# fredli74/hashbox

Hardware: AMD Instinct MI355X
Metric: device-resident GiB/s chunked+hashed at 1/2/4/8 MI355X; % HBM roofline (higher is better)
Workload: dtype u8

## Files before the change

hashbox_amd/csrc/hbx_kernels.hip:

```cpp
#include <type_traits>
#include <utility>

#include "hbx_device.h"

using namespace hbx;

namespace {

constexpr int kK1Threads = 1024;

struct RunAgg {
  uint32_t ah, jh, af, jf;
};
__device__ __forceinline__ RunAgg run_aggregates(const uint32_t (&v)[16]) {
  RunAgg r;
  uint32_t a = 0, j = 0;
#pragma unroll
  for (int k = 0; k < 8; k++) {
    a = dot4(v[k], 0x01010101u, a);
    j = dot4(v[k], jw(k), j);
  }
  r.ah = a;
  r.jh = j;
#pragma unroll
// ... 670 lines not shown
    }
    md5_compress(h, m);
  }
}

__device__ void md5_block_at(const uint8_t* c, uint32_t len, uint32_t (&h)[4], uint32_t b) {
  const uint32_t sh = (uint32_t)reinterpret_cast<uintptr_t>(c) & 3u;
  g_u32* va = gptr32(c - sh);
  const uint32_t base = b ? 16u * b - 2u : 0u;
  uint32_t v[17];
#pragma unroll
  for (int j = 0; j < 17; j++) v[j] = va[base + (uint32_t)j];
  uint32_t m[16];
#pragma unroll
  for (int j = 0; j < 16; j++) {
    const uint32_t dw = alignbyte(v[j + 1], v[j], sh);
    const uint32_t d0 = j >= 2 ? alignbyte(v[j - 1], v[j - 2], sh) : 0u;
    m[j] = b ? dw : (j == 0 ? 0u : j == 1 ? bswap32(len) : d0);
  }
  md5_compress(h, m);
}

template <int G>
struct Coop {
  static constexpr uint32_t C = 64u / G;
  static constexpr uint32_t Row = 16u * G + 16u;
  static constexpr uint32_t Half = 64u * Row;
  static constexpr uint32_t WaveLds = 2u * Half;
  static constexpr uint32_t BPS = G / 4u;
};
constexpr uint32_t kCoopWaveLds = Coop<16>::WaveLds;

__device__ __forceinline__ uint64_t shfl64(uint64_t v, uint32_t src_lane) {
  const int lo = __builtin_amdgcn_ds_bpermute((int)(src_lane << 2), (int)(uint32_t)v);
  const int hi = __builtin_amdgcn_ds_bpermute((int)(src_lane << 2), (int)(uint32_t)(v >> 32));
  return ((uint64_t)(uint32_t)hi << 32) | (uint32_t)lo;
}

template <int G>
__device__ __forceinline__ void coop_write(uint8_t* wl, uint32_t wr, uint32_t half, const u32x4 (&Gs)[G]) {
#pragma unroll
  for (int q = 0; q < G; q++)
    *reinterpret_cast<u32x4*>(wl + wr + half * Coop<G>::Half + Coop<G>::C * Coop<G>::Row * (uint32_t)q) = Gs[q];
}

template <int G>
__device__ __forceinline__ void coop_load(u32x4 (&Gs)[G], const uint64_t (&Q)[G], uint32_t st, uint32_t t,
                                          uint32_t ngr) {
  const uint32_t g = min((uint32_t)G * st + t, ngr - 1u);
  const uint64_t off = 16ull * (g - t);
#pragma unroll
  for (int q = 0; q < G; q++) Gs[q] = md5_load(gptr128(Q[q] + off));
}

template <int G>
__device__ __forceinline__ void coop_hash(const uint8_t* wl, uint32_t rd, uint32_t half, uint32_t s, uint32_t R,
                                          uint32_t (&h)[4]) {
  const uint8_t* hb = wl + rd + half * Coop<G>::Half;
#pragma unroll
  for (int u = 0; u < (int)Coop<G>::BPS; u++) {
    const uint32_t blk = Coop<G>::BPS * s + (uint32_t)u;
    if (blk >= R) break;
    u32x4 W[4];
#pragma unroll
    for (int i = 0; i < 4; i++) W[i] = *reinterpret_cast<const u32x4*>(hb + 16u * (4u * u + (uint32_t)i));
    const uint32_t m[16] = {W[0].x, W[0].y, W[0].z, W[0].w, W[1].x, W[1].y, W[1].z, W[1].w,
                            W[2].x, W[2].y, W[2].z, W[2].w, W[3].x, W[3].y, W[3].z, W[3].w};
    md5_compress(h, m);
  }
}

template <int G>
__device__ void md5_coop(uint8_t* wl, const uint8_t* c, uint32_t (&h)[4], uint32_t b1, uint32_t R) {
  static_assert(G == 16, "stage of 4 blocks");
  const uint32_t lane = threadIdx.x & 63u;
  const uint64_t S = reinterpret_cast<uint64_t>(c) + 64ull * b1 - 8ull;
  const uint32_t ngr = 4u * R;
  const uint32_t t = lane % (uint32_t)G, sub = lane / (uint32_t)G;
  uint64_t Q[G];
#pragma unroll
  for (int q = 0; q < G; q++) Q[q] = shfl64(S, Coop<G>::C * (uint32_t)q + sub) + 16ull * t;
  const uint32_t wr = sub * Coop<G>::Row + 16u * t;
  const uint32_t rd = lane * Coop<G>::Row;
  const uint32_t nst = (ngr + (uint32_t)G - 1u) / (uint32_t)G;
  constexpr uint32_t BPS = Coop<G>::BPS;
  u32x4 GA[G], GB[G];
  coop_load<G>(GA, Q, 0u, t, ngr);
  coop_load<G>(GB, Q, 1u, t, ngr);
  coop_write<G>(wl, wr, 0u, GA);
  coop_load<G>(GA, Q, 2u, t, ngr);
  auto stage = [&](auto half_c, uint32_t s, u32x4(&Gn)[G]) {
    constexpr uint32_t HALF = decltype(half_c)::value;
    coop_write<G>(wl, wr, HALF ^ 1u, Gn);
    coop_load<G>(Gn, Q, min(s + 3u, nst - 1u), t, ngr);
    coop_hash<G>(wl, rd, HALF, s, R, h);
  };
  for (uint32_t s = 0; BPS * s < R; s += 2u) {
    stage(std::integral_constant<uint32_t, 0>{}, s, GB);
    stage(std::integral_constant<uint32_t, 1>{}, s + 1u, GA);
  }
}

}

struct alignas(16) Chain {
  uint64_t src;
  uint32_t len;
  uint32_t next;
  uint32_t h[4];
  uint64_t out;
  uint64_t pad;
};
constexpr uint32_t kChainDone = 0xFFFFFFFFu;
constexpr uint32_t kBudgetAll = 0xFFFFFFFFu;

#ifndef HBX_SLICE_REM_FIRST
#define HBX_SLICE_REM_FIRST 1
#endif
__device__ __forceinline__ uint32_t slice_cnt(uint32_t left, uint32_t budget) {
  if (left <= budget) return left;
  return HBX_SLICE_REM_FIRST ? (left - 1u) % budget + 1u : budget;
}

struct OrderEntry {
  uint64_t chain;
  uint32_t rem;
  uint32_t pad;
};
constexpr uint32_t kPlanBins = 1024u;
__device__ __forceinline__ uint32_t order_bin(uint32_t cnt, uint32_t budget) {
  const uint32_t ref = min(budget, (uint32_t)(kMaxBlock >> 6) + 1u);
  const uint32_t c = min(cnt, ref);
  return (ref - c) * (kPlanBins - 1u) / ref;
}
__device__ __forceinline__ uint32_t plan_bin(const OrderEntry& o, uint32_t budget, uint32_t abins, uint32_t ashift) {
  const uint32_t cnt = slice_cnt(o.rem - 1u, budget);
  if (!abins) return order_bin(cnt, budget);
  if (cnt == budget) return (uint32_t)((reinterpret_cast<const Chain*>(o.chain)->src >> ashift) % abins);
  const uint32_t ref = min(budget, (uint32_t)(kMaxBlock >> 6) + 1u);
  const uint32_t c = min(cnt, ref);
  return abins + (ref - c) * (kPlanBins - 1u - abins) / ref;
}

constexpr uint32_t kPlanLanesPerFile = 16u;

extern "C" __global__ __launch_bounds__(256) void hbx_k2r_new_chains(
    uint32_t n_files, const uint8_t* __restrict__ arena, const uint64_t* __restrict__ file_off,
    const uint64_t* __restrict__ cut_base, const uint64_t* __restrict__ cut_ends,
    const uint32_t* __restrict__ cut_count, uint32_t* __restrict__ ids, Chain* __restrict__ run,
    OrderEntry* __restrict__ fresh, uint32_t* __restrict__ cnt, const uint64_t* __restrict__ first_start) {
  const uint32_t w = blockIdx.x * 256u + threadIdx.x;
  if (w >= n_files * kPlanLanesPerFile) return;
  const uint32_t f = w / kPlanLanesPerFile;
  const uint64_t cb = cut_base[f];
  const uint32_t k = cut_count[f];
  const uint64_t base = reinterpret_cast<uint64_t>(arena + file_off[f]);
  const uint64_t s0 = first_start ? first_start[f] : 0ull;
  for (uint32_t i = w % kPlanLanesPerFile; i < k; i += kPlanLanesPerFile) {
    const uint64_t start = i ? cut_ends[cb + i - 1] : s0;
    const uint64_t e = cut_ends[cb + i];
    Chain ch;
    ch.src = base + start;
    ch.len = (uint32_t)(e - start);
    ch.next = 0u;
    ch.h[0] = 0x67452301u;
    ch.h[1] = 0xefcdab89u;
    ch.h[2] = 0x98badcfeu;
    ch.h[3] = 0x10325476u;
    ch.out = reinterpret_cast<uint64_t>(ids + 4u * (cb + i));
    ch.pad = 0ull;
    const uint32_t slot = atomicAdd(cnt, 1u);
    run[slot] = ch;
    OrderEntry o;
    o.chain = reinterpret_cast<uint64_t>(run + slot);
    o.rem = ((ch.len + 8u) >> 6) + 1u;
    o.pad = 0u;
    fresh[slot] = o;
  }
}

constexpr int kPlanThreads = 1024;
static_assert(kPlanThreads == (int)kPlanBins, "one planner thread per bin");
constexpr uint32_t kPlanGroups = 32u;
constexpr int kMaxFresh = 8;
struct FreshSet {
  const OrderEntry* f[kMaxFresh];
  const uint32_t* n[kMaxFresh];
  uint32_t k, pad;
};

extern "C" __global__ __launch_bounds__(kPlanThreads) void hbx_k2c_plan(
    const OrderEntry* __restrict__ prev, const uint32_t* __restrict__ n_prev_p, uint32_t bprev,
    FreshSet fs, uint32_t budget, OrderEntry* __restrict__ out, uint32_t* __restrict__ n_out,
    uint32_t* __restrict__ gh, uint32_t phase) {
  const uint32_t abins = (phase >> 8) & 0xfffu;
  const uint32_t ashift = phase >> 24;
  phase &= 0xffu;
  __shared__ uint32_t hist[kPlanBins], pos[kPlanBins], wsum[kPlanThreads / 64];
  const uint32_t tid = threadIdx.x;
  const uint32_t gt = blockIdx.x * kPlanThreads + tid, gn = gridDim.x * kPlanThreads;
  const uint32_t n_prev = prev ? *n_prev_p : 0u;
  uint32_t fend[kMaxFresh];
  uint32_t n_all = n_prev;
#pragma unroll
  for (int i = 0; i < kMaxFresh; i++) {
    n_all += (uint32_t)i < fs.k ? *fs.n[i] : 0u;
    fend[i] = n_all;
  }
  auto entry = [&](uint32_t e) {
    OrderEntry o;
    if (e < n_prev) {
      o = prev[e];
      o.rem = o.rem - 1u <= bprev ? 0u : o.rem - slice_cnt(o.rem - 1u, bprev);
    } else {
      const OrderEntry* f = fs.f[0];
      uint32_t base = n_prev;
#pragma unroll
      for (int i = 1; i < kMaxFresh; i++)
        if (e >= fend[i - 1]) {
          f = fs.f[i];
          base = fend[i - 1];
        }
      o = f[e - base];
    }
    return o;
  };
  hist[tid] = 0u;
  __syncthreads();
  for (uint32_t e = gt; e < n_all; e += gn) {
    const OrderEntry o = entry(e);
    if (o.rem) atomicAdd(&hist[plan_bin(o, budget, abins, ashift)], 1u);
  }
  __syncthreads();
  if (phase == 0u) {
    if (hist[tid]) atomicAdd(&gh[tid], hist[tid]);
    return;
  }
  {
    const uint32_t v = gh[tid];
    const uint32_t inc = wave_incl_sum(v);
    if ((tid & 63u) == 63u) wsum[tid >> 6] = inc;
    __syncthreads();
    uint32_t before = 0u;
    for (uint32_t wv = 0; wv < (tid >> 6); wv++) before += wsum[wv];
    const uint32_t mine = hist[tid];
    pos[tid] = before + inc - v + (mine ? atomicAdd(&gh[kPlanBins + tid], mine) : 0u);
    if (blockIdx.x == 0 && tid == kPlanThreads - 1) {
      *n_out = before + inc;
      n_out[1] = 0u;
      n_out[2] = 0u;
    }
  }
  __syncthreads();
  for (uint32_t e = gt; e < n_all; e += gn) {
    const OrderEntry o = entry(e);
    if (o.rem) out[atomicAdd(&pos[plan_bin(o, budget, abins, ashift)], 1u)] = o;
  }
}

constexpr uint32_t kCoopMinBudget = 8u;
constexpr int kK3Threads = 256;
constexpr uint32_t kK3WaveLds = Coop<16>::WaveLds;

__device__ __forceinline__ uint32_t k3p_flag(uint32_t* p) {
  return __hip_atomic_load(p, __ATOMIC_RELAXED, __HIP_MEMORY_SCOPE_WORKGROUP);
}
__device__ __forceinline__ void k3p_wait_ge(uint32_t* p, uint32_t want) {
  for (;;) {
    const uint32_t v = (uint32_t)__builtin_amdgcn_readfirstlane((int)k3p_flag(p));
    if ((int32_t)(v - want) >= 0) break;
    __builtin_amdgcn_s_sleep(1);
  }
  asm volatile("" ::: "memory");
}
__device__ __forceinline__ void k3p_wait_ge(uint32_t* p, uint32_t want, uint32_t& polls, bool spin) {
  for (;;) {
    const uint32_t v = (uint32_t)__builtin_amdgcn_readfirstlane((int)k3p_flag(p));
    if ((int32_t)(v - want) >= 0) break;
    polls++;
    if (!spin) __builtin_amdgcn_s_sleep(1);
  }
  asm volatile("" ::: "memory");
}
__device__ __forceinline__ void k3p_publish(uint32_t* p, uint32_t v) {
  asm volatile("s_waitcnt lgkmcnt(0)" ::: "memory");
  if ((threadIdx.x & 63u) == 0u) __hip_atomic_store(p, v, __ATOMIC_RELAXED, __HIP_MEMORY_SCOPE_WORKGROUP);
}

__device__ __forceinline__ void k3p_consume(uint8_t* wl, uint32_t* flags, uint32_t S, uint32_t Rr, uint32_t (&h)[4],
                                            uint32_t& polls, bool spin) {
  const uint32_t row = (uint32_t)(uintptr_t)(wl + (threadIdx.x & 63u) * Coop<16>::Row);
  auto stage_at = [&](uint32_t k) { return row + ((S + k) & 1u) * Coop<16>::Half; };
  auto next_wait = [&](uint32_t a, u32x4(&N)[4], u32x4(&W)[4]) {
    asm volatile(
        "ds_read_b128 %0, %8\n\t"
        "ds_read_b128 %1, %8 offset:16\n\t"
        "ds_read_b128 %2, %8 offset:32\n\t"
        "ds_read_b128 %3, %8 offset:48\n\t"
        "s_waitcnt lgkmcnt(4)"
        : "=&v"(N[0]), "=&v"(N[1]), "=&v"(N[2]), "=&v"(N[3]), "+v"(W[0]), "+v"(W[1]), "+v"(W[2]), "+v"(W[3])
        : "v"(a)
        : "memory");
  };
  auto hash = [&](const u32x4(&W)[4]) {
    const uint32_t m[16] = {W[0].x, W[0].y, W[0].z, W[0].w, W[1].x, W[1].y, W[1].z, W[1].w,
                            W[2].x, W[2].y, W[2].z, W[2].w, W[3].x, W[3].y, W[3].z, W[3].w};
    md5_compress(h, m);
  };
  const uint32_t nst = (4u * Rr + 15u) / 16u;
  u32x4 WA[4], WB[4];
  k3p_wait_ge(&flags[0], S + 1u, polls, spin);
  asm volatile(
      "ds_read_b128 %0, %4\n\t"
      "ds_read_b128 %1, %4 offset:16\n\t"
      "ds_read_b128 %2, %4 offset:32\n\t"
      "ds_read_b128 %3, %4 offset:48"
      : "=&v"(WA[0]), "=&v"(WA[1]), "=&v"(WA[2]), "=&v"(WA[3])
      : "v"(stage_at(0u))
      : "memory");
  for (uint32_t k = 0; k + 1u < nst; k++) {
    const uint32_t a0 = stage_at(k);
    next_wait(a0 + 64u, WB, WA);
    hash(WA);
    next_wait(a0 + 128u, WA, WB);
    hash(WB);
    next_wait(a0 + 192u, WB, WA);
    hash(WA);
    k3p_wait_ge(&flags[0], S + k + 2u, polls, spin);
    next_wait(stage_at(k + 1u), WA, WB);
    hash(WB);
    asm volatile("" ::: "memory");
    if ((threadIdx.x & 63u) == 0u) __hip_atomic_store(&flags[1], S + k + 1u, __ATOMIC_RELAXED, __HIP_MEMORY_SCOPE_WORKGROUP);
  }
  asm volatile("s_waitcnt lgkmcnt(0)" : "+v"(WA[0]), "+v"(WA[1]), "+v"(WA[2]), "+v"(WA[3]) : : "memory");
  hash(WA);
  const uint8_t* last = wl + (threadIdx.x & 63u) * Coop<16>::Row + ((S + nst - 1u) & 1u) * Coop<16>::Half;
  for (uint32_t u = 1; 4u * (nst - 1u) + u < Rr; u++) {
    u32x4 W[4];
#pragma unroll
    for (int i = 0; i < 4; i++) W[i] = *reinterpret_cast<const u32x4*>(last + 64u * u + 16u * i);
    hash(W);
  }
}

struct K3Group {
  uint64_t src;
  uint32_t next;
  uint32_t cnt, R;
  bool active;
};
__device__ __forceinline__ K3Group k3_group(const OrderEntry* __restrict__ order, uint32_t n_total, uint32_t g,
                                            uint32_t budget) {
  const uint32_t lane = threadIdx.x & 63u;
  const uint32_t k = 64u * g + lane;
  K3Group G;
  G.active = k < n_total;
  const OrderEntry o = order[G.active ? k : 64u * g];
  const Chain* chp = reinterpret_cast<const Chain*>(o.chain);
  G.src = chp->src;
  const uint32_t left = o.rem - 1u;
  G.next = ((chp->len + 8u) >> 6) - left;
  G.cnt = G.active ? slice_cnt(left, budget) : 0u;
  G.R = ~wave_max_all(G.active ? ~G.cnt : 0u);
  return G;
}

template <int SETS = 2>
__device__ __forceinline__ uint32_t k3p_produce(uint8_t* wl, uint32_t* flags, uint32_t S, uint64_t src, uint32_t Rr) {
  const uint32_t lane = threadIdx.x & 63u;
  const uint32_t t = lane % 16u, sub = lane / 16u;
  const uint32_t wr = sub * Coop<16>::Row + 16u * t;
  const uint32_t ngr = 4u * Rr, nst = (ngr + 15u) / 16u;
  uint64_t Q[16];
#pragma unroll
  for (int q = 0; q < 16; q++) Q[q] = shfl64(src, 4u * (uint32_t)q + sub) + 16ull * t;
  u32x4 GA[16], GB[16];
  coop_load<16>(GA, Q, 0u, t, ngr);
  coop_load<16>(GB, Q, min(1u, nst - 1u), t, ngr);
  if (SETS == 3) {
    u32x4 GC[16];
    coop_load<16>(GC, Q, min(2u, nst - 1u), t, ngr);
    auto put = [&](uint32_t x, u32x4 (&G)[16]) {
      k3p_wait_ge(&flags[1], x < 2u ? S : S + x - 1u);
      coop_write<16>(wl, wr, (S + x) & 1u, G);
      k3p_publish(&flags[0], S + x + 1u);
      coop_load<16>(G, Q, min(x + 3u, nst - 1u), t, ngr);
    };
    for (uint32_t s = 0; s < nst; s += 3u) {
      put(s, GA);
      if (s + 1u < nst) put(s + 1u, GB);
      if (s + 2u < nst) put(s + 2u, GC);
    }
    return nst;
  }
  for (uint32_t s = 0; s < nst; s += 2u) {
    k3p_wait_ge(&flags[1], s < 2u ? S : S + s - 1u);
    coop_write<16>(wl, wr, (S + s) & 1u, GA);
    k3p_publish(&flags[0], S + s + 1u);
    coop_load<16>(GA, Q, min(s + 2u, nst - 1u), t, ngr);
    if (s + 1u < nst) {
      k3p_wait_ge(&flags[1], s + 1u < 2u ? S : S + s);
      coop_write<16>(wl, wr, (S + s + 1u) & 1u, GB);
      k3p_publish(&flags[0], S + s + 2u);
      coop_load<16>(GB, Q, min(s + 3u, nst - 1u), t, ngr);
    }
  }
  return nst;
}

constexpr uint32_t kItemExit = 0xFFFFFFFFu;
constexpr uint32_t kItemSpinTicks = 20000000u;

struct K3Lane {
  Chain* chp;
  const uint8_t* src;
  uint32_t next;
  uint32_t len, b0, cnt;
  bool finish, live;
  uint32_t h[4];
};
template <bool ITEMS>
__device__ __forceinline__ K3Lane k3_lane(const OrderEntry* __restrict__ order, uint32_t n_total, uint32_t g,
                                          uint32_t part, uint32_t budget, uint32_t per_part) {
  const uint32_t lane = threadIdx.x & 63u;
  const uint32_t k = 64u * g + lane;
  const bool active = k < n_total;
  K3Lane L;
  if constexpr (!ITEMS) {
    const OrderEntry o = order[active ? k : 64u * g];
    L.chp = reinterpret_cast<Chain*>(o.chain);
    const Chain ch = *L.chp;
    const uint32_t left = o.rem - 1u;
    L.next = ((ch.len + 8u) >> 6) - left;
    L.len = active ? ch.len : 0u;
    L.b0 = active ? L.next : 0u;
    L.cnt = active ? slice_cnt(left, budget) : 0u;
    L.finish = active && left <= budget;
    L.live = active;
    L.src = reinterpret_cast<const uint8_t*>(ch.src);
    L.h[0] = ch.h[0];
    L.h[1] = ch.h[1];
    L.h[2] = ch.h[2];
    L.h[3] = ch.h[3];
  } else {
    const OrderEntry o = order[active ? k : 64u * g];
    L.chp = reinterpret_cast<Chain*>(o.chain);
    Chain ch = *L.chp;
    ch.next = __hip_atomic_load(&L.chp->next, __ATOMIC_RELAXED, __HIP_MEMORY_SCOPE_AGENT);
#pragma unroll
    for (int i = 0; i < 4; i++) ch.h[i] = __hip_atomic_load(&L.chp->h[i], __ATOMIC_RELAXED, __HIP_MEMORY_SCOPE_AGENT);
    const uint32_t nfull = (ch.len + 8u) >> 6;
    const uint32_t total = slice_cnt(o.rem - 1u, budget);
    const uint32_t start = nfull - (o.rem - 1u);
    const uint64_t lo64 = (uint64_t)part * per_part;
    const uint32_t lo = lo64 < total ? (uint32_t)lo64 : total;
    const uint32_t hi = (uint64_t)lo + per_part < total ? lo + per_part : total;
    const uint32_t last = total ? (total - 1u) / per_part : 0u;
    L.live = active && part <= last && ch.next != kChainDone;
    L.len = L.live ? ch.len : 0u;
    L.b0 = L.live ? ch.next : 0u;
    L.cnt = L.live ? hi - lo : 0u;
    L.finish = L.live && part == last && start + total == nfull;
    (void)start;
    L.src = reinterpret_cast<const uint8_t*>(ch.src);
    L.next = ch.next;
    L.h[0] = ch.h[0];
    L.h[1] = ch.h[1];
    L.h[2] = ch.h[2];
    L.h[3] = ch.h[3];
    const uint32_t mx = wave_max_all(L.cnt);
    if (mx) {
      const int Ls = __builtin_ctzll(__builtin_amdgcn_ballot_w64(L.cnt == mx));
      const uint64_t sa = reinterpret_cast<uint64_t>(L.src);
      const uint64_t ss = ((uint64_t)(uint32_t)__builtin_amdgcn_readlane((int)(sa >> 32), Ls) << 32) |
                          (uint32_t)__builtin_amdgcn_readlane((int)(uint32_t)sa, Ls);
      const uint32_t ns = (uint32_t)__builtin_amdgcn_readlane((int)L.next, Ls);
      if (L.cnt == 0u && !L.finish) {
        L.src = reinterpret_cast<const uint8_t*>(ss);
        L.next = ns;
      }
    }
  }
  return L;
}
template <bool ITEMS>
__device__ __forceinline__ uint32_t k3_wave_R(const K3Lane& L) {
  if constexpr (!ITEMS) return ~wave_max_all(L.live ? ~L.cnt : 0u);
  const uint32_t m = wave_max_all((L.cnt || L.finish) ? ~L.cnt : 0u);
  return m ? ~m : 0u;
}

__device__ __forceinline__ uint32_t k3q_pop(uint32_t* __restrict__ qc, const uint64_t* __restrict__ q, uint32_t G,
                                            uint32_t total, uint32_t tag, uint32_t* __restrict__ err) {
  uint32_t item = kItemExit;
  if ((threadIdx.x & 63u) == 0u) {
    const uint32_t sl = __hip_atomic_fetch_add(&qc[0], 1u, __ATOMIC_RELAXED, __HIP_MEMORY_SCOPE_AGENT);
    if (sl < G) {
      item = sl;
    } else if (sl < total) {
      const uint64_t t0 = __builtin_amdgcn_s_memrealtime();
      for (;;) {
        const uint64_t v = __hip_atomic_load(&q[sl - G], __ATOMIC_RELAXED, __HIP_MEMORY_SCOPE_AGENT);
        if ((uint32_t)(v >> 32) == tag) {
          item = (uint32_t)v;
          break;
        }
        if (__builtin_amdgcn_s_memrealtime() - t0 > (uint64_t)kItemSpinTicks) {
          if (err) __hip_atomic_store(err, 1u, __ATOMIC_RELAXED, __HIP_MEMORY_SCOPE_SYSTEM);
          break;
        }
        __builtin_amdgcn_s_sleep(2);
      }
    }
  }
  return (uint32_t)__builtin_amdgcn_readlane((int)item, 0);
}
__device__ __forceinline__ void k3q_push(uint32_t* __restrict__ qc, uint64_t* __restrict__ q, uint32_t tag,
                                         uint32_t item) {
  asm volatile("s_waitcnt vmcnt(0) lgkmcnt(0)" ::: "memory");
  if ((threadIdx.x & 63u) == 0u) {
    const uint32_t t = __hip_atomic_fetch_add(&qc[1], 1u, __ATOMIC_RELAXED, __HIP_MEMORY_SCOPE_AGENT);
    __hip_atomic_store(&q[t], ((uint64_t)tag << 32) | item, __ATOMIC_RELAXED, __HIP_MEMORY_SCOPE_AGENT);
  }
}

template <int SETS>
__device__ void k3p_producer(uint8_t* wl, uint32_t* flags, const OrderEntry* __restrict__ order,
                             const uint32_t* __restrict__ n_order, uint32_t budget, uint32_t g0, uint32_t nwaves) {
  const uint32_t n_total = *n_order;
  const uint32_t groups = (n_total + 63u) / 64u;
  uint32_t S = 0;
  for (uint32_t g = g0; g < groups; g += nwaves) {
    const K3Group G = k3_group(order, n_total, g, budget);
    if (G.R < kCoopMinBudget) continue;
    S += k3p_produce<SETS>(wl, flags, S, G.src + 64ull * (G.next + 1u) - 8ull, G.R - 1u);
  }
  asm volatile("s_waitcnt vmcnt(0)" ::: "memory");
}
__device__ void k3q_producer(uint8_t* wl, uint32_t* flags, const OrderEntry* __restrict__ order,
                             const uint32_t* __restrict__ n_order, uint32_t budget, uint32_t parts,
                             uint32_t per_part) {
  const uint32_t n_total = *n_order;
  const uint32_t G = (n_total + 63u) / 64u;
  uint32_t S = 0;
  for (uint32_t seq = 1;; seq++) {
    k3p_wait_ge(&flags[3], seq);
    const uint32_t item = (uint32_t)__builtin_amdgcn_readfirstlane((int)k3p_flag(&flags[2]));
    if (item == kItemExit) break;
    const K3Lane L = k3_lane<true>(order, n_total, item % G, item / G, budget, per_part);
    const uint32_t R = k3_wave_R<true>(L);
    if (R < kCoopMinBudget) continue;
    S += k3p_produce(wl, flags, S, reinterpret_cast<uint64_t>(L.src) + 64ull * (L.next + 1u) - 8ull, R - 1u);
  }
  (void)parts;
  asm volatile("s_waitcnt vmcnt(0)" ::: "memory");
}

struct K3Queue {
  uint32_t* qc;
  uint64_t* q;
  uint32_t tag, parts;
  uint32_t* err;
};
template <bool PROD, bool ITEMS = false>
__device__ __forceinline__ void k3_body(
    uint8_t* wl, const OrderEntry* __restrict__ order, const uint32_t* __restrict__ n_order, uint32_t budget,
    uint32_t* __restrict__ started, uint32_t t_first, uint32_t t_last, uint64_t* __restrict__ tslot,
    uint64_t* __restrict__ probe, uint32_t* flags = nullptr, K3Queue Q = K3Queue{}, bool spin = false) {
  static_assert(PROD || !ITEMS, "items need the producer waves");
  __builtin_amdgcn_s_setprio(3);
  if (started && threadIdx.x == 0) {
    const uint32_t tk = __hip_atomic_fetch_add(started, 1u, __ATOMIC_RELEASE, __HIP_MEMORY_SCOPE_AGENT);
    if (tslot && tk == t_first) tslot[0] = __builtin_amdgcn_s_memrealtime();
  }
  const uint32_t wave = (uint32_t)__builtin_amdgcn_readfirstlane((int)(threadIdx.x >> 6));
  const uint32_t n_total = *n_order;
  const uint32_t groups = (n_total + 63u) / 64u;
  const uint32_t nwaves = gridDim.x * (kK3Threads / 64);
  const uint32_t g0 = blockIdx.x * (kK3Threads / 64) + wave;
  const uint32_t per_part = ITEMS ? (budget == kBudgetAll ? kBudgetAll : (budget + Q.parts - 1u) / Q.parts) : 0u;
  const uint64_t pt0 = probe ? __builtin_amdgcn_s_memrealtime() : 0ull;
  uint64_t pt1 = 0ull, pc1 = 0ull, pc2 = 0ull, pt2 = 0ull;
  uint32_t pR = 0u, pmax = 0u;
  uint32_t S = 0;
  uint32_t seq = 0;
  uint32_t polls = 0;
  bool first = true;
  for (uint32_t g = g0;; g += nwaves) {
    uint32_t part = 0u, item = 0u;
    if constexpr (ITEMS) {
      item = g0 < groups ? k3q_pop(Q.qc, Q.q, groups, groups * Q.parts, Q.tag, Q.err) : kItemExit;
      if ((threadIdx.x & 63u) == 0u) {
        __hip_atomic_store(&flags[2], item, __ATOMIC_RELAXED, __HIP_MEMORY_SCOPE_WORKGROUP);
      }
      k3p_publish(&flags[3], ++seq);
      if (item == kItemExit) break;
      g = item % groups;
      part = item / groups;
    } else {
      if (g >= groups) break;
    }
    K3Lane L = k3_lane<ITEMS>(order, n_total, g, part, budget, per_part);
    uint32_t(&h)[4] = L.h;
    const uint8_t* src = L.src;
    const uint32_t len = L.len, b0 = L.b0, cnt = L.cnt;
    const bool finish = L.finish;
    const uint32_t R = k3_wave_R<ITEMS>(L);
    if (R >= kCoopMinBudget) {
      md5_block_at(src, len, h, L.next);
      if (probe && first) {
        pt1 = __builtin_amdgcn_s_memrealtime();
        pc1 = __builtin_amdgcn_s_memtime();
        pR = R;
        pmax = wave_max_all(cnt);
      }
      if constexpr (PROD) {
        k3p_consume(wl, flags, S, R - 1u, h, polls, spin);
        S += (4u * (R - 1u) + 15u) / 16u;
      } else {
        md5_coop<16>(wl, src, h, L.next + 1u, R - 1u);
      }
      if (probe && first) {
        pc2 = __builtin_amdgcn_s_memtime();
        pt2 = __builtin_amdgcn_s_memrealtime();
      }
      uint32_t pos = b0 + R, rem = cnt ? cnt - R : 0u;
      for (int round = 0; round < 4; round++) {
        const uint32_t mx = wave_max_all(rem ? ~rem : 0u);
        if (mx == 0u || ~mx < kCoopMinBudget) break;
        const uint32_t R2 = ~mx;
        const bool part_ = rem != 0u;
        const int Lr = __builtin_ctzll(__builtin_amdgcn_ballot_w64(part_));
        const uint64_t s_sh = ((uint64_t)(uint32_t)__builtin_amdgcn_readlane((int)(reinterpret_cast<uint64_t>(src) >> 32), Lr) << 32) |
                              (uint32_t)__builtin_amdgcn_readlane((int)(uint32_t)reinterpret_cast<uint64_t>(src), Lr);
        const uint32_t p_sh = (uint32_t)__builtin_amdgcn_readlane((int)pos, Lr);
        uint32_t hk[4] = {h[0], h[1], h[2], h[3]};
        md5_coop<16>(wl, part_ ? src : reinterpret_cast<const uint8_t*>(s_sh), hk, part_ ? pos : p_sh, R2);
        if (part_) {
          h[0] = hk[0];
          h[1] = hk[1];
          h[2] = hk[2];
          h[3] = hk[3];
          pos += R2;
          rem -= R2;
        }
      }
      md5_run<PROD ? 4 : HBX_MD5_RING>(src, len, h, pos, rem, finish);
      if constexpr (PROD) k3p_publish(&flags[1], S);
    } else {
      md5_run<PROD ? 4 : HBX_MD5_RING>(src, len, h, b0, cnt, finish);
    }
    if constexpr (!ITEMS) {
      if (finish) {
        *(__attribute__((address_space(1))) u32x4*)L.chp->out = u32x4{h[0], h[1], h[2], h[3]};
        L.chp->next = kChainDone;
      } else if (L.live) {
        *reinterpret_cast<uint4*>(&L.chp->h[0]) = make_uint4(h[0], h[1], h[2], h[3]);
        L.chp->next = b0 + cnt;
      }
    } else {
      if (finish) {
        *(__attribute__((address_space(1))) u32x4*)L.chp->out = u32x4{h[0], h[1], h[2], h[3]};
        __hip_atomic_store(&L.chp->next, kChainDone, __ATOMIC_RELAXED, __HIP_MEMORY_SCOPE_AGENT);
      } else if (L.live && cnt) {
#pragma unroll
        for (int i = 0; i < 4; i++) __hip_atomic_store(&L.chp->h[i], h[i], __ATOMIC_RELAXED, __HIP_MEMORY_SCOPE_AGENT);
        __hip_atomic_store(&L.chp->next, b0 + cnt, __ATOMIC_RELAXED, __HIP_MEMORY_SCOPE_AGENT);
      }
    }
    if constexpr (ITEMS) {
      if (part + 1u < Q.parts) k3q_push(Q.qc, Q.q, Q.tag, item + groups);
    }
    first = false;
  }
  if (probe && (threadIdx.x & 63u) == 0u) {
    uint64_t* p = probe + 8u * (blockIdx.x * (kK3Threads / 64) + wave);
    const uint32_t hw = __builtin_amdgcn_s_getreg(4 | (31 << 11));
    const uint32_t xcc = __builtin_amdgcn_s_getreg(20 | (31 << 11)) & 0xfu;
    p[0] = pt0;
    p[1] = pt1 | ((uint64_t)xcc << 56);
    p[2] = __builtin_amdgcn_s_memrealtime();
    p[3] = (uint64_t)min(pR, 0xffffu) | ((uint64_t)min(pmax, 0xffffu) << 16) | ((uint64_t)hw << 32);
    p[4] = pc1;
    p[5] = pc2;
    p[6] = pt2;
    p[7] = (pR ? pR - 1u : 0u) | ((uint64_t)polls << 32);
  }
  if (started && tslot && (threadIdx.x & 63u) == 0u) {
    const uint32_t tk = __hip_atomic_fetch_add(started + 1, 1u, __ATOMIC_RELEASE, __HIP_MEMORY_SCOPE_AGENT);
    if (tk == t_last) tslot[1] = __builtin_amdgcn_s_memrealtime();
  }
}


extern "C" __global__ __launch_bounds__(kK3Threads, 1) void hbx_k3_block_md5(
    const OrderEntry* __restrict__ order, const uint32_t* __restrict__ n_order, uint32_t budget,
    uint32_t* __restrict__ started, uint32_t t_first, uint32_t t_last, uint64_t* __restrict__ tslot,
    uint64_t* __restrict__ probe) {
  __shared__ __attribute__((aligned(16))) uint8_t k3_lds[kK3Threads / 64][kK3WaveLds];
  const uint32_t wave = (uint32_t)__builtin_amdgcn_readfirstlane((int)(threadIdx.x >> 6));
  k3_body<false>(k3_lds[wave], order, n_order, budget, started, t_first, t_last, tslot, probe);
}

constexpr int kK3PThreads = 512;
extern "C" __global__ __launch_bounds__(kK3PThreads, 1) void hbx_k3p_block_md5(
    const OrderEntry* __restrict__ order, const uint32_t* __restrict__ n_order, uint32_t budget,
    uint32_t* __restrict__ started, uint32_t t_first, uint32_t t_last, uint64_t* __restrict__ tslot,
    uint64_t* __restrict__ probe, uint32_t psets) {
  const bool spin = (psets & 0x100u) != 0u;
  psets &= 0xffu;
  __shared__ __attribute__((aligned(16))) uint8_t k3_lds[4][kK3WaveLds];
  __shared__ uint32_t k3_flags[4][2];
  const uint32_t wave = (uint32_t)__builtin_amdgcn_readfirstlane((int)(threadIdx.x >> 6));
  const uint32_t pair = wave & 3u;
  if (threadIdx.x < 8u) k3_flags[threadIdx.x >> 1][threadIdx.x & 1u] = 0u;
  __syncthreads();
  if (wave < 4u) {
    k3_body<true>(k3_lds[pair], order, n_order, budget, started, t_first, t_last, tslot, probe, k3_flags[pair],
                  K3Queue{}, spin);
  } else {
    __builtin_amdgcn_s_setprio(2);
    if (psets == 3u)
      k3p_producer<3>(k3_lds[pair], k3_flags[pair], order, n_order, budget, blockIdx.x * 4u + pair, gridDim.x * 4u);
    else
      k3p_producer<2>(k3_lds[pair], k3_flags[pair], order, n_order, budget, blockIdx.x * 4u + pair, gridDim.x * 4u);
  }
}

extern "C" __global__ __launch_bounds__(kK3PThreads, 1) void hbx_k3q_block_md5(
    const OrderEntry* __restrict__ order, const uint32_t* __restrict__ n_order, uint32_t budget,
    uint32_t* __restrict__ started, uint32_t t_first, uint32_t t_last, uint64_t* __restrict__ tslot,
    uint64_t* __restrict__ probe, uint32_t* __restrict__ qc, uint64_t* __restrict__ q, uint32_t tag, uint32_t parts,
    uint32_t* __restrict__ err) {
  __shared__ __attribute__((aligned(16))) uint8_t k3_lds[4][kK3WaveLds];
  __shared__ uint32_t k3_flags[4][4];
  const uint32_t wave = (uint32_t)__builtin_amdgcn_readfirstlane((int)(threadIdx.x >> 6));
  const uint32_t pair = wave & 3u;
  if (threadIdx.x < 16u) k3_flags[threadIdx.x >> 2][threadIdx.x & 3u] = 0u;
  __syncthreads();
  if (wave < 4u) {
    k3_body<true, true>(k3_lds[pair], order, n_order, budget, started, t_first, t_last, tslot, probe, k3_flags[pair],
                        K3Queue{qc, q, tag, parts, err});
  } else {
    __builtin_amdgcn_s_setprio(2);
    const uint32_t per_part = budget == kBudgetAll ? kBudgetAll : (budget + parts - 1u) / parts;
    k3q_producer(k3_lds[pair], k3_flags[pair], order, n_order, budget, parts, per_part);
  }
}

__device__ __forceinline__ void meta_copy(const uint4* __restrict__ src, uint4* __restrict__ dst, uint32_t n) {
  for (uint32_t i = blockIdx.x * blockDim.x + threadIdx.x; i < n; i += gridDim.x * blockDim.x) {
    uint32_t* p = const_cast<uint32_t*>(reinterpret_cast<const uint32_t*>(src + i));
    uint4 v;
    v.x = __hip_atomic_load(p + 0, __ATOMIC_RELAXED, __HIP_MEMORY_SCOPE_SYSTEM);
    v.y = __hip_atomic_load(p + 1, __ATOMIC_RELAXED, __HIP_MEMORY_SCOPE_SYSTEM);
    v.z = __hip_atomic_load(p + 2, __ATOMIC_RELAXED, __HIP_MEMORY_SCOPE_SYSTEM);
    v.w = __hip_atomic_load(p + 3, __ATOMIC_RELAXED, __HIP_MEMORY_SCOPE_SYSTEM);
    dst[i] = v;
  }
}
extern "C" __global__ __launch_bounds__(256) void hbx_k1_gate_meta(const uint32_t* __restrict__ started,
                                                                   uint32_t target, uint32_t limit,
                                                                   uint32_t poll, const uint4* __restrict__ msrc,
                                                                   uint4* __restrict__ mdst, uint32_t n16) {
  meta_copy(msrc, mdst, n16);
  if (!poll || blockIdx.x != 0 || threadIdx.x != 0) return;
  const uint64_t t0 = __builtin_amdgcn_s_memrealtime();
  for (;;) {
    const uint32_t v = __hip_atomic_load(started, __ATOMIC_ACQUIRE, __HIP_MEMORY_SCOPE_AGENT);
    if ((int32_t)(v - target) >= 0) break;
    if (__builtin_amdgcn_s_memrealtime() - t0 > (uint64_t)limit) break;
    __builtin_amdgcn_s_sleep(2);
  }
}
extern "C" __global__ __launch_bounds__(64) void hbx_k1_gate(const uint32_t* __restrict__ started,
                                                              uint32_t target, uint32_t limit) {
  if (threadIdx.x != 0) return;
  const uint64_t t0 = __builtin_amdgcn_s_memrealtime();
  for (;;) {
    const uint32_t v = __hip_atomic_load(started, __ATOMIC_ACQUIRE, __HIP_MEMORY_SCOPE_AGENT);
    if ((int32_t)(v - target) >= 0) break;
    if (__builtin_amdgcn_s_memrealtime() - t0 > (uint64_t)limit) break;
    __builtin_amdgcn_s_sleep(2);
  }
}

extern "C" __global__ __launch_bounds__(256) void hbx_meta_fetch(const uint4* __restrict__ src,
                                                                 uint4* __restrict__ dst, uint32_t n) {
  for (uint32_t i = blockIdx.x * 256u + threadIdx.x; i < n; i += gridDim.x * 256u) {
    uint32_t* p = const_cast<uint32_t*>(reinterpret_cast<const uint32_t*>(src + i));
    uint4 v;
    v.x = __hip_atomic_load(p + 0, __ATOMIC_RELAXED, __HIP_MEMORY_SCOPE_SYSTEM);
    v.y = __hip_atomic_load(p + 1, __ATOMIC_RELAXED, __HIP_MEMORY_SCOPE_SYSTEM);
    v.z = __hip_atomic_load(p + 2, __ATOMIC_RELAXED, __HIP_MEMORY_SCOPE_SYSTEM);
    v.w = __hip_atomic_load(p + 3, __ATOMIC_RELAXED, __HIP_MEMORY_SCOPE_SYSTEM);
    dst[i] = v;
  }
}

extern "C" __global__ __launch_bounds__(256) void hbx_result_push(const uint4* __restrict__ src,
                                                                  uint4* __restrict__ dst, uint64_t n) {
  for (uint64_t i = (uint64_t)blockIdx.x * 256u + threadIdx.x; i < n; i += (uint64_t)gridDim.x * 256u)
    dst[i] = src[i];
  __threadfence_system();
}

constexpr uint32_t kK4Window = 1024u;

extern "C" __global__ __launch_bounds__(64) void hbx_k4_content_id(
    uint32_t n_files, const uint64_t* __restrict__ cut_base, const uint32_t* __restrict__ cut_count,
    const uint32_t* __restrict__ ids, uint32_t* __restrict__ content_ids,
    int32_t* __restrict__ content_type, uint32_t window) {
  __shared__ uint4 win[kK4Window];
  const uint32_t f = blockIdx.x;
  if (f >= n_files) return;
  const uint32_t k = cut_count[f];
  const uint4* id = reinterpret_cast<const uint4*>(ids) + cut_base[f];
  uint4* co = reinterpret_cast<uint4*>(content_ids) + f;
  if (k <= 1u) {
    if (threadIdx.x == 0) {
      *co = k ? id[0] : make_uint4(0u, 0u, 0u, 0u);
      content_type[f] = k ? 2 : 0;
    }
    return;
  }
  uint32_t w0 = 0xFFFFFFFFu;
  auto get = [&](uint32_t i) -> uint4 {
    if (i < w0 || i - w0 >= window) {
      __syncthreads();
      for (uint32_t t = threadIdx.x; t < window && i + t < k; t += 64u) win[t] = id[i + t];
      __syncthreads();
      w0 = i;
    }
    return win[i - w0];
  };
  const uint32_t nw = 12u * k + 4u;
  const uint32_t T = 4u * nw;
  const uint32_t nblk = (T + 9u + 63u) / 64u;
  uint32_t h[4];
  md5_init(h);
  for (uint32_t b = 0; b < nblk; b++) {
    uint32_t m[16];
#pragma unroll
    for (int i = 0; i < 16; i++) {
      const uint32_t j = 16u * b + (uint32_t)i;
      uint32_t v;
      if (j == 0u) {
        v = bswap32(k);
      } else if (j <= 4u * k) {
        const uint4 q = get((j - 1u) >> 2);
        const uint32_t r = (j - 1u) & 3u;
        v = r == 0 ? q.x : r == 1 ? q.y : r == 2 ? q.z : q.w;
      } else if (j == 4u * k + 1u) {
        v = bswap32(8u + 32u * k);
      } else if (j == 4u * k + 2u) {
        v = bswap32(0x6663686Eu);
      } else if (j == 4u * k + 3u) {
        v = bswap32(k);
      } else if (j < nw) {
        const uint32_t t = j - (4u * k + 4u);
        const uint32_t r = t & 7u;
        if (r < 4u) {
          const uint4 q = get(t >> 3);
          v = r == 0 ? q.x : r == 1 ? q.y : r == 2 ? q.z : q.w;
        } else {
          v = 0u;
        }
      } else if (j == nw) {
        v = 0x80u;
      } else {
        v = 0u;
      }
      m[i] = v;
    }
    if (b + 1 == nblk) {
      const uint64_t bits = (uint64_t)T * 8ull;
      m[14] = (uint32_t)bits;
      m[15] = (uint32_t)(bits >> 32);
    }
    md5_compress(h, m);
  }
  if (threadIdx.x == 0) {
    *co = make_uint4(h[0], h[1], h[2], h[3]);
    content_type[f] = 3;
  }
}

extern "C" __global__ __launch_bounds__(64) void hbx_k5_md5_raw(const uint8_t* __restrict__ msg,
                                                                 uint32_t n, uint32_t* __restrict__ out) {
  if (threadIdx.x != 0) return;
  uint32_t h[4];
  md5_init(h);
  const uint32_t nblk = (n + 9u + 63u) / 64u;
  for (uint32_t b = 0; b < nblk; b++) {
    uint32_t m[16];
#pragma unroll
    for (int i = 0; i < 16; i++) {
      uint32_t v = 0u;
#pragma unroll
      for (int y = 0; y < 4; y++) {
        const uint32_t p = 64u * b + 4u * (uint32_t)i + (uint32_t)y;
        const uint32_t by = p < n ? msg[p] : (p == n ? 0x80u : 0u);
        v |= by << (8 * y);
      }
      m[i] = v;
    }
    if (b + 1 == nblk) {
      const uint64_t bits = (uint64_t)n * 8ull;
      m[14] = (uint32_t)bits;
      m[15] = (uint32_t)(bits >> 32);
    }
    md5_compress(h, m);
  }
  out[0] = h[0];
  out[1] = h[1];
  out[2] = h[2];
  out[3] = h[3];
}

extern "C" __global__ __launch_bounds__(64) void hbx_k5r_md5_run(const uint8_t* __restrict__ msg, uint32_t n,
                                                                 uint32_t* __restrict__ out) {
  uint32_t h[4];
  md5_init(h);
  const uint32_t* w = reinterpret_cast<const uint32_t*>(msg);
  uint32_t m[16];
#pragma unroll
  for (int i = 0; i < 16; i++) m[i] = w[i];
  md5_compress(h, m);
  md5_run<>(msg + 8, n - 8u, h, 1u, (n >> 6) - 1u, true);
  if (threadIdx.x == 0) {
    out[0] = h[0];
    out[1] = h[1];
    out[2] = h[2];
    out[3] = h[3];
  }
// ... 138 lines not shown
```

Measured before the change: 2378.

## Piggyback producer flag read on LDS loads and use power-of-two coop tail rounds

The consumer loop now reads the producer flag in the same LDS batch as the next message block, and calls the spin-wait only when the observed stage is not yet ready. This aims to remove a separate polling round-trip from the steady-state hashing loop. The cooperative tail loop also changes from up to four rounds sized by the minimum remaining length to descending power-of-two budgets, where every lane with enough remaining bytes takes part. That should let more residual work go through the wide cooperative path instead of the per-lane ring, at the cost of more rounds for small remainders.

```diff
diff --git a/hashbox_amd/csrc/hbx_kernels.hip b/hashbox_amd/csrc/hbx_kernels.hip
--- a/hashbox_amd/csrc/hbx_kernels.hip
+++ b/hashbox_amd/csrc/hbx_kernels.hip
@@ -996,6 +996,22 @@
         : "v"(a)
         : "memory");
   };
+  const uint32_t fa = (uint32_t)(uintptr_t)&flags[0];
+  auto next_wait_flag = [&](uint32_t a, u32x4(&N)[4], u32x4(&W)[4]) {
+    uint32_t f;
+    asm volatile(
+        "ds_read_b32 %8, %10\n\t"
+        "ds_read_b128 %0, %9\n\t"
+        "ds_read_b128 %1, %9 offset:16\n\t"
+        "ds_read_b128 %2, %9 offset:32\n\t"
+        "ds_read_b128 %3, %9 offset:48\n\t"
+        "s_waitcnt lgkmcnt(4)"
+        : "=&v"(N[0]), "=&v"(N[1]), "=&v"(N[2]), "=&v"(N[3]), "+v"(W[0]), "+v"(W[1]), "+v"(W[2]), "+v"(W[3]),
+          "=&v"(f)
+        : "v"(a), "v"(fa)
+        : "memory");
+    return (uint32_t)__builtin_amdgcn_readfirstlane((int)f);
+  };
   auto hash = [&](const u32x4(&W)[4]) {
     const uint32_t m[16] = {W[0].x, W[0].y, W[0].z, W[0].w, W[1].x, W[1].y, W[1].z, W[1].w,
                             W[2].x, W[2].y, W[2].z, W[2].w, W[3].x, W[3].y, W[3].z, W[3].w};
@@ -1018,9 +1034,9 @@
     hash(WA);
     next_wait(a0 + 128u, WA, WB);
     hash(WB);
-    next_wait(a0 + 192u, WB, WA);
+    const uint32_t seen = next_wait_flag(a0 + 192u, WB, WA);
     hash(WA);
-    k3p_wait_ge(&flags[0], S + k + 2u, polls, spin);
+    if ((int32_t)(seen - (S + k + 2u)) < 0) k3p_wait_ge(&flags[0], S + k + 2u, polls, spin);
     next_wait(stage_at(k + 1u), WA, WB);
     hash(WB);
     asm volatile("" ::: "memory");
@@ -1319,12 +1335,13 @@
         pt2 = __builtin_amdgcn_s_memrealtime();
       }
       uint32_t pos = b0 + R, rem = cnt ? cnt - R : 0u;
-      for (int round = 0; round < 4; round++) {
-        const uint32_t mx = wave_max_all(rem ? ~rem : 0u);
-        if (mx == 0u || ~mx < kCoopMinBudget) break;
-        const uint32_t R2 = ~mx;
-        const bool part_ = rem != 0u;
-        const int Lr = __builtin_ctzll(__builtin_amdgcn_ballot_w64(part_));
+      const uint32_t rmax = wave_max_all(rem);
+      for (uint32_t R2 = rmax >= kCoopMinBudget ? 0x80000000u >> __builtin_clz(rmax) : 0u; R2 >= kCoopMinBudget;
+           R2 >>= 1) {
+        const bool part_ = rem >= R2;
+        const uint64_t who = __builtin_amdgcn_ballot_w64(part_);
+        if (who == 0ull) continue;
+        const int Lr = __builtin_ctzll(who);
         const uint64_t s_sh = ((uint64_t)(uint32_t)__builtin_amdgcn_readlane((int)(reinterpret_cast<uint64_t>(src) >> 32), Lr) << 32) |
                               (uint32_t)__builtin_amdgcn_readlane((int)(uint32_t)reinterpret_cast<uint64_t>(src), Lr);
         const uint32_t p_sh = (uint32_t)__builtin_amdgcn_readlane((int)pos, Lr);
```

Result: no change. 2376 (-0.1%).
